# yang-z-03/scd-resnet

Hardware: AMD Instinct MI355X
Metric: 512x512 images/sec training, centerOffsetRes10, at 1/2/4/8 MI355X (higher is better)
Workload: dtype bf16; 1 GPU; centerOffsetRes10 train step (fwd+focal/L1 loss+bwd+Adam, DDP over RCCL), 512x512 synthetic SCD tiles; model=centerOffsetRes10, global_batch=32, step_issue=eager launches, per_gpu_batch=32, parallelism=dp1, image_size=512

## Files before the change

### include/scdhip.h

```cpp
#ifndef SCDHIP_H
#define SCDHIP_H
#include <stddef.h>
#include <stdint.h>

#ifdef __cplusplus
extern "C" {
#endif

#define SCD_DT_F32 0
#define SCD_DT_BF16 1
#define SCD_DT_F16 2

#define SCD_ERR_ARG 9001

#define SCD_MAX_TAPS 16
#define SCD_MAX_PHASES 4
#define SCD_STAT_REPLICAS 64

typedef struct scd_gemm_phase {
    int Qh, Qw, rho_h, rho_w, ntaps;
    int dh[SCD_MAX_TAPS], dw[SCD_MAX_TAPS], wt[SCD_MAX_TAPS];
} scd_gemm_phase;

int scd_conv_gemm(int dtype, const void* x, const void* w, void* y, const float* bias, double* stats,
                  int N, int Hi, int Wi, int Ci, int Ho, int Wo, int Co, int in_stride, int out_stride,
                  int wrow, int relu, int accumulate, int nphase, const scd_gemm_phase* phases,
                  void* stream);

int scd_conv_dgrad_s2(int dtype, const void* dy, const void* w3, void* dx, int N, int Hq, int Wq, int Cg, int Cin,
                      int accumulate, void* stream);
int scd_conv_gemm_bnbwd(int dtype, const void* x, const void* w, void* y, int N, int Hi, int Wi, int Ci, int Ho,
                        int Wo, int Co, int in_stride, int out_stride, int wrow, int nphase,
                        const scd_gemm_phase* phases, const void* bn_y, const float* mean, const float* invstd,
                        const float* relu_scale, const float* relu_shift, double* bn_stats, void* stream);
int scd_conv_gemm_heads(int dtype, const void* x, const void* w, void* hid, const float* bias, int N, int H,
                        int W, int Ci, int nh, const int* od, const float* const* w1, const float* const* b1,
                        float* const* outs, void* stream);
int scd_conv_gemm_heads_keep(int dtype, const void* x, const void* w, void* hid, const float* bias, int N, int H,
                             int W, int Ci, int nh, const int* od, const float* const* w1, const float* const* b1,
                             float* const* outs, const unsigned char* keep, int keep_cols, void* stream);

size_t scd_conv_wgrad_workspace(int Cg, int T, int Ci, int nsplit);
int scd_conv_wgrad_nsplit(int dtype, long M, int Cg, int T, int Ci);
int scd_conv_wgrad_nsplit2(int dtype, long M, int Ho, int Wo, int Cg, int T, int Ci);
int scd_conv_wgrad(int dtype, const void* g, const void* x, float* ws, int nsplit,
                   int N, int Ho, int Wo, int Cg, int Hi, int Wi, int Ci, int in_stride,
                   int T, const int* dh, const int* dw, void* stream);
int scd_wgrad_reduce(const float* ws, int nsplit, int Cg, int T, int Ci, int r0, int r1, int cvalid,
                     long ld_n, long ld_c, long ld_t, float* dst, int accumulate, float alpha, void* stream);
int scd_wgrad_reduce_rows(const float* ws, int nsplit, int Cg, int T, int Ci, int nslices, const int* r0,
                          const int* r1, const long* ld_n, const long* ld_c, const long* ld_t, float* const* dst,
                          int cvalid, int accumulate, float alpha, void* stream);

int scd_pack_weight(int dtype, const float* w, void* out, int A, int B, int T, int mode, int ldp,
                    int row_off, void* stream);

int scd_pad_channels(int dtype, const void* src, long rows, int C, int Cp, void* dst, void* stream);

typedef struct scd_pack_desc {
    const float* w;
    void* out;
    long start;
    int A, B, T, mode, ldp, row_off, a_off, a_tot;
} scd_pack_desc;
int scd_pack_weights_batched(int dtype, const scd_pack_desc* descs, int n, long total, void* stream);

int scd_im2col_stem(int dtype, const float* x, void* cols, int N, int H, int W, int Ho, int Wo, int kh,
                    int kw, int stride, int pad, int Kpad, void* stream);

int scd_stem_conv_fwd(int dtype, const float* x, const void* wpk, void* y, double* stats, int N, int H, int W,
                      int Ho, int Wo, void* stream);
int scd_stem_conv_wgrad_nsplit(long M);
int scd_stem_conv_wgrad(int dtype, const void* dy, const void* ybn, const float* coef, const float* x, float* ws,
                        int nsplit, int N, int H, int W, int Ho, int Wo, void* stream);
int scd_stem_bwd_nsplit(void);
int scd_stem_bwd_fused(int dtype, const void* dout, const uint8_t* argmax, const void* y, const float* scale,
                       const float* shift, const float* mean, const float* invstd, const float* x, double* stats,
                       float* ws, int nsplit, float* tg, int N, int H, int W, int Ho, int Wo, void* stream);
int scd_stem_bwd_combine(int dtype, const float* tg, const void* wpk, const float* coef, float* dst, int accumulate,
                         float alpha, void* stream);

int scd_stats_collapse(double* stats, int nrep, int C, void* stream);
int scd_stats_collapse_to(double* stats, int nrep, int C, double* out, void* stream);
int scd_bn_finalize(double* stats, int nrep, int C, double count, const float* gamma,
                    const float* beta, float* running_mean, float* running_var, int64_t* num_batches,
                    float momentum, float eps, float* mean, float* invstd, float* scale, float* shift,
                    void* stream);
#define SCD_BN_FIN_MAX 4
typedef struct scd_bn_fin_args {
    double* stats;
    int nrep, C;
    double count;
    const float* gamma;
    const float* beta;
    float* running_mean;
    float* running_var;
    int64_t* num_batches;
    float momentum, eps;
    float* mean;
    float* invstd;
    float* scale;
    float* shift;
} scd_bn_fin_args;
int scd_bn_finalize_n(const scd_bn_fin_args* layers, int n, void* stream);
int scd_bn_apply(int dtype, const void* y, void* out, int C, long total, const float* scale,
                 const float* shift, const void* res, const float* rscale, const float* rshift,
                 int relu, void* stream);
int scd_bn_bwd_reduce(int dtype, const void* dout, const void* mask, const void* y, const float* relu_scale,
                      const float* relu_shift, const float* mean, const float* invstd, int C, long total,
                      double* stats, void* stream);
int scd_bn_bwd_finalize(double* stats, int nrep, int C, double count, const float* gamma,
                        const float* mean, const float* invstd, float* dgamma, float* dbeta,
                        float gscale, float* coef, void* stream);
typedef struct scd_bn_bwd_fin_args {
    double* stats;
    int nrep, C;
    double count;
    const float* gamma;
    const float* mean;
    const float* invstd;
    float* dgamma;
    float* dbeta;
    float gscale;
    float* coef;
} scd_bn_bwd_fin_args;
int scd_bn_bwd_finalize_n(const scd_bn_bwd_fin_args* layers, int n, void* stream);
int scd_bn_bwd_apply(int dtype, const void* dout, const void* mask, const void* y, const float* relu_scale,
                     const float* relu_shift, const float* coef, int C, long total, void* dy, void* dz,
                     void* stream);

int scd_bn_bwd_reduce2(int dtype, const void* dout, const void* mask, const void* ya, const void* yb,
                       const float* mean_a, const float* invstd_a, const float* mean_b, const float* invstd_b, int C,
                       long total, double* stats_a, double* stats_b, void* stream);
int scd_bn_bwd_apply2(int dtype, const void* dout, const void* mask, const void* ya, const void* yb,
                      const float* coef_a, const float* coef_b, int C, long total, void* dya, void* dyb, void* stream);
// ... 122 lines not shown
```

### scd-resnet_amd/csrc/conv_gemm.hip

```cpp
#include <stdlib.h>

#include <algorithm>
#include <type_traits>

#include "scd_common.h"

#ifndef SCD_ABLATE
#define SCD_ABLATE 0
#endif
#ifndef L1P_SWAP
#define L1P_SWAP 1
#endif
#ifndef S1X1_FULLROW
#define S1X1_FULLROW 1
#endif
#ifndef S1X1_STG
#define S1X1_STG 1
#endif
#ifndef S1X1_UA2
#define S1X1_UA2 1
#endif
#ifndef WGRAD_OCC
#define WGRAD_OCC 2
#endif
// ... 3591 lines not shown
    fill_params(p, dy, w3, dx, nullptr, nullptr, N, Hq, Wq, Cg, Hq, Wq, Co, 1, 1, 4 * Cg, 0, accumulate);
    p.shuf = 1;
    scd_gemm_phase ph;
    ph.Qh = Hq; ph.Qw = Wq; ph.rho_h = 0; ph.rho_w = 0; ph.ntaps = 4;
    for (int t = 0; t < 4; ++t) { ph.dh[t] = t >> 1; ph.dw[t] = t & 1; ph.wt[t] = t; }
    return conv_gemm_launch(dtype, p, 1, &ph, stream);
}

extern "C" int scd_conv_gemm_heads(int dtype, const void* x, const void* w, void* hid, const float* bias, int N,
                                   int H, int W, int Ci, int nh, const int* od, const float* const* w1,
                                   const float* const* b1, float* const* outs, void* stream) {
    SCD_F16_FWD(scd_conv_gemm_heads, x, w, hid, bias, N, H, W, Ci, nh, od, w1, b1, outs, stream);
    return scd_conv_gemm_heads_keep(dtype, x, w, hid, bias, N, H, W, Ci, nh, od, w1, b1, outs, nullptr, 0, stream);
}

extern "C" int scd_conv_gemm_heads_keep(int dtype, const void* x, const void* w, void* hid, const float* bias, int N,
                                        int H, int W, int Ci, int nh, const int* od, const float* const* w1,
                                        const float* const* b1, float* const* outs, const unsigned char* keep,
                                        int keep_cols, void* stream) {
    SCD_F16_FWD(scd_conv_gemm_heads_keep, x, w, hid, bias, N, H, W, Ci, nh, od, w1, b1, outs, keep, keep_cols, stream);
    if (nh < 1 || nh > 4 || (keep && (keep_cols < 0 || keep_cols % 128))) return SCD_ERR_ARG;
    GemmParams p;
    fill_params(p, x, w, hid, bias, nullptr, N, H, W, Ci, H, W, nh * 128, 1, 1, 9 * Ci, 1, 0);
    if (keep) { p.hid_keep = keep; p.hid_cols = keep_cols; }
    p.head_on = 1;
    for (int h = 0; h < nh; ++h) {
        if (od[h] < 1 || od[h] > 4) return SCD_ERR_ARG;
        p.head_od[h] = od[h]; p.head_w[h] = w1[h]; p.head_b[h] = b1[h]; p.head_out[h] = outs[h];
    }
    scd_gemm_phase ph;
    ph.Qh = H; ph.Qw = W; ph.rho_h = 0; ph.rho_w = 0; ph.ntaps = 9;
    for (int t = 0; t < 9; ++t) { ph.dh[t] = t / 3 - 1; ph.dw[t] = t % 3 - 1; ph.wt[t] = t; }
    return conv_gemm_launch(dtype, p, 1, &ph, stream);
}

extern "C" size_t scd_conv_wgrad_workspace(int Cg, int T, int Ci, int nsplit) {
    return (size_t)nsplit * Cg * T * Ci * sizeof(float);
}

static bool wgrad_fastx() {
    static int mode = -2;
    if (mode == -2) { const char* e = getenv("SCD_WGRAD_FASTX"); mode = e ? atoi(e) : 1; }
    return mode != 0;
}

static void wgrad_tile(int dtype, long M, int Cg, int& tm, int& tn) {
    (void)dtype; (void)M;
    if (Cg <= 64) { tm = 64; tn = 256; }
    else { tm = 128; tn = 128; }
}

static bool wgrad_use_pp2(int dtype, long M, int Ho, int Wo, int Cg) {
    static int mode = -2;
    if (mode == -2) { const char* e = getenv("SCD_WGRAD_PP2"); mode = e ? atoi(e) : 1; }
    const bool stage_ok = Wo % 64 == 0 || (Wo >= 8 && 64 % Wo == 0);
    return mode && dtype == SCD_DT_BF16 && Cg >= 128 && stage_ok && ((long)Ho * Wo) % 64 == 0 && M >= 64 * 64;
}

static bool wgrad_use_l1(int dtype, long M, int Ho, int Wo, int Cg, int T, int Ci) {
    static int mode = -2;
    if (mode == -2) { const char* e = getenv("SCD_WGRAD_L1"); mode = e ? atoi(e) : 1; }
    return mode && dtype == SCD_DT_BF16 && Cg == 64 && Ci == 64 && T == 9 && Wo % 64 == 0 && M % 64 == 0 &&
           (long)Ho * Wo * 64 <= (1L << 30) && M >= 64;
}

static int wgrad_l1_nsplit(long M) {
    static long cap = -2;
    if (cap == -2) { const char* e = getenv("SCD_WGRAD_L1_NSPLIT"); cap = e ? atol(e) : 192; }
    return (int)std::max(1L, std::min(cap, M / 64 / 16));
}

static int wgrad_pp2_win(int Cg) {
    if (Cg % 256 == 0) return 256;
    if (Cg % 192 == 0) return 192;
    return Cg < 256 ? 128 : 256;
}

static bool wgrad_nsmodel() {
    static int mode = -2;
    if (mode == -2) { const char* e = getenv("SCD_WGRAD_NSMODEL"); mode = e ? atoi(e) : 1; }
    return mode != 0;
}

static long wgrad_ns_model(long M, long tiles, int slots, int kp, double stage_us, double epi_us, double slab_bytes,
                           long ns_max, bool any_ns = false) {
    static double slab_rate = -1.0;
    if (slab_rate < 0) { const char* e = getenv("SCD_WGRAD_SLAB_TBPS"); slab_rate = (e ? atof(e) : 0.8) * 1e6; }
    long best = 8;
    double bt = 1e30;
    const long step = any_ns ? 1 : 8;
    for (long ns = step; ns <= std::max(8L, ns_max); ns += step) {
        const long stages = cdiv(cdiv(M, ns), (long)kp);
        const long rounds = cdiv(tiles * ns, (long)slots);
        const double t = rounds * (stages * stage_us + epi_us) + ns * slab_bytes / slab_rate;
        if (t < bt * 0.995) { bt = t; best = ns; }
    }
    return best;
}

static int wgrad_pp2_nsplit(long M, int Cg, int KK) {
    const int win = wgrad_pp2_win(Cg);
    const long tiles = (long)(Cg / win) * cdiv(KK, 256);
    const long cap_px = std::max(8L, M / 512 / 8 * 8);
    const long cap_mem = std::max(8L, (256L << 20) / std::max(1L, 4L * Cg * KK) / 8 * 8);
    if (wgrad_nsmodel()) {
        const double stage_us = 2.0 * win * 256 * 64 / 4.3e6;
        const double epi_us = 4.0 * win * 256 / (5.0e6 / 256);
        static int slots = -1;
        if (slots < 0) { const char* e = getenv("SCD_WGRAD_SLOTS"); slots = e ? std::max(8, atoi(e)) : 256; }
        const long ns = wgrad_ns_model(M, tiles, slots, 64, stage_us, epi_us, 4.0 * Cg * KK, std::min(cap_px, cap_mem),
                                       tiles >= 24);
        return (int)ns;
    }
    long ns = std::max(8L, (512L / tiles + 4) / 8 * 8);
    ns = std::min(ns, cap_px);
    ns = std::min(ns, cap_mem);
    return (int)ns;
}

extern "C" int scd_conv_wgrad_nsplit2(int dtype, long M, int Ho, int Wo, int Cg, int T, int Ci) {
    SCD_F16_FWD(scd_conv_wgrad_nsplit2, M, Ho, Wo, Cg, T, Ci);
    if (wgrad_use_l1(dtype, M, Ho, Wo, Cg, T, Ci)) return wgrad_l1_nsplit(M);
    if (wgrad_use_pp2(dtype, M, Ho, Wo, Cg)) return wgrad_pp2_nsplit(M, Cg, T * Ci);
    return scd_conv_wgrad_nsplit(dtype, M, Cg, T, Ci);
}

extern "C" int scd_conv_wgrad_nsplit(int dtype, long M, int Cg, int T, int Ci) {
    SCD_F16_FWD(scd_conv_wgrad_nsplit, M, Cg, T, Ci);
    int tm, tn;
    wgrad_tile(dtype, M, Cg, tm, tn);
    const long tiles = (long)cdiv(Cg, tm) * cdiv((long)T * Ci, tn);
    if (wgrad_nsmodel() && M >= 8 * 1024) {
        const int KP = dtype == SCD_DT_BF16 ? 64 : 32;
        const int slots = tm == 64 ? 256 : 512;
        const double stage_us = 2.0 * tm * tn * KP / (2.4e6 * 256 / slots);
        const double epi_us = 4.0 * tm * tn / (5.0e6 / slots);
        const long cap_px = std::max(8L, M / 1024 / 8 * 8);
        const long cap_mem = std::max(8L, (256L << 20) / std::max(1L, 4L * Cg * T * Ci) / 8 * 8);
        const long ns = wgrad_ns_model(M, tiles, slots, KP, stage_us, epi_us, 4.0 * Cg * T * Ci,
                                       std::min(cap_px, cap_mem));
        return (int)ns;
    }
    long ns = std::max(1L, std::min(1024L / std::max(1L, tiles), M / 1024));
    ns = std::max(1L, std::min(ns, (256L << 20) / std::max(1L, 4L * Cg * T * Ci)));
    if (ns >= 8) ns = ns / 8 * 8;
    return (int)ns;
}

extern "C" int scd_conv_wgrad(int dtype, const void* g, const void* x, float* ws, int nsplit, int N, int Ho, int Wo,
                              int Cg, int Hi, int Wi, int Ci, int in_stride, int T, const int* dh, const int* dw,
                              void* stream) {
    SCD_F16_FWD(scd_conv_wgrad, g, x, ws, nsplit, N, Ho, Wo, Cg, Hi, Wi, Ci, in_stride, T, dh, dw, stream);
    const int EPC = dtype == SCD_DT_BF16 ? 8 : 4;
    if (T < 1 || T > SCD_MAX_TAPS || Ci % EPC != 0 || Cg % EPC != 0 || nsplit < 1) return SCD_ERR_ARG;
    WgradParams p;
    p.g = (const char*)g; p.x = (const char*)x; p.ws = ws;
    p.N = N; p.Ho = Ho; p.Wo = Wo; p.Cg = Cg; p.Hi = Hi; p.Wi = Wi; p.Ci = Ci; p.is = in_stride; p.T = T;
    p.cg0 = 0; p.cgn = Cg;
    p.KK = T * Ci;
    {
        const int esz = dtype == SCD_DT_BF16 ? 2 : 4;
        const long gb = (long)N * Ho * Wo * Cg * esz, xb = (long)N * Hi * Wi * Ci * esz;
        if (gb >= (1L << 31) - 64 || xb >= (1L << 31) - 64) return SCD_ERR_ARG;
        p.gbytes = (int)gb;
        p.xbytes = (int)xb;
    }
    for (int t = 0; t < SCD_MAX_TAPS; ++t) { p.dh[t] = t < T ? dh[t] : 0; p.dw[t] = t < T ? dw[t] : 0; }
    const long M = (long)N * Ho * Wo;
    int chunk = cdiv(M, nsplit);
    chunk = (chunk + 63) / 64 * 64;
    p.chunk = chunk;
    if (wgrad_use_l1(dtype, M, Ho, Wo, Cg, T, Ci) && in_stride == 1 && Hi == Ho && Wi == Wo) {
        bool std_taps = true;
        for (int t = 0; t < 9; ++t) std_taps &= dh[t] == t / 3 - 1 && dw[t] == t % 3 - 1;
        if (std_taps) {
            p.nsplit = nsplit;
            hipLaunchKernelGGL(conv_wgrad_l1_kernel, dim3(nsplit), dim3(512), 0, (hipStream_t)stream, p);
            SCD_RETURN_LAUNCH();
        }
    }
    if (wgrad_use_pp2(dtype, M, Ho, Wo, Cg) && chunk % 64 == 0) {
        hipStream_t st = (hipStream_t)stream;
        p.ntn = cdiv(p.KK, 256);
        p.nsplit = nsplit;
        const int n8 = nsplit;
        const int win = wgrad_pp2_win(Cg);
        p.cg0 = 0;
        p.cgn = Cg / win * win;
        p.ntm = Cg / win;
        if (win == 256) hipLaunchKernelGGL((conv_wgrad_pp2_kernel<4>), dim3(p.ntm * p.ntn * n8), dim3(512), 0, st, p);
        else if (win == 192) hipLaunchKernelGGL((conv_wgrad_pp2_kernel<3>), dim3(p.ntm * p.ntn * n8), dim3(512), 0, st, p);
        else hipLaunchKernelGGL((conv_wgrad_pp2_kernel<2>), dim3(p.ntm * p.ntn * n8), dim3(512), 0, st, p);
        hipError_t e = hipGetLastError();
        if (e != hipSuccess || Cg % win == 0) return (int)e;
// ... 4 lines not shown
        p.ntm = cdiv(p.cgn, BM);
        p.ntn = cdiv(p.KK, BN);
        const int fx = !(wgrad_fastx() && ((long)Ho * Wo) % 64 == 0) ? 0 : (Wo % 64 == 0 ? 1 : 2);
        dim3 grid(p.ntm * p.ntn * n8);
        if (BM == 64) {
            if (fx == 1) hipLaunchKernelGGL((conv_wgrad_kernel<h16, 64, 256, 1>), grid, dim3(256), 0, st, p);
            else if (fx == 2) hipLaunchKernelGGL((conv_wgrad_kernel<h16, 64, 256, 2>), grid, dim3(256), 0, st, p);
            else hipLaunchKernelGGL((conv_wgrad_kernel<h16, 64, 256, 0>), grid, dim3(256), 0, st, p);
        } else {
            if (fx == 1) hipLaunchKernelGGL((conv_wgrad_kernel<h16, 128, 128, 1>), grid, dim3(256), 0, st, p);
            else hipLaunchKernelGGL((conv_wgrad_kernel<h16, 128, 128, 0>), grid, dim3(256), 0, st, p);
        }
        SCD_RETURN_LAUNCH();
    }
    int BM, BN;
    wgrad_tile(dtype, M, Cg, BM, BN);
    p.ntm = cdiv(Cg, BM);
    p.ntn = cdiv(p.KK, BN);
    p.nsplit = nsplit;
    dim3 grid(p.ntm * p.ntn * nsplit);
    hipStream_t st = (hipStream_t)stream;
    if (dtype == SCD_DT_BF16 || dtype == SCD_DT_F32) {
        const int KP = dtype == SCD_DT_BF16 ? 64 : 32;
        const bool fastok = wgrad_fastx() && ((long)Ho * Wo) % KP == 0 && chunk % KP == 0;
        const int fx = !fastok ? 0 : (Wo % KP == 0 ? 1 : (KP % Wo == 0 ? 2 : 0));
        if (dtype == SCD_DT_BF16) {
            if (Cg <= 64) {
                if (fx == 1) hipLaunchKernelGGL((conv_wgrad_kernel<h16, 64, 256, 1>), grid, dim3(256), 0, st, p);
                else if (fx == 2) hipLaunchKernelGGL((conv_wgrad_kernel<h16, 64, 256, 2>), grid, dim3(256), 0, st, p);
                else hipLaunchKernelGGL((conv_wgrad_kernel<h16, 64, 256, 0>), grid, dim3(256), 0, st, p);
            } else {
                if (fx == 1) hipLaunchKernelGGL((conv_wgrad_kernel<h16, 128, 128, 1>), grid, dim3(256), 0, st, p);
                else hipLaunchKernelGGL((conv_wgrad_kernel<h16, 128, 128, 0>), grid, dim3(256), 0, st, p);
            }
        } else {
            if (Cg <= 64) {
                if (fx == 1) hipLaunchKernelGGL((conv_wgrad_kernel<float, 64, 256, 1>), grid, dim3(256), 0, st, p);
                else if (fx == 2) hipLaunchKernelGGL((conv_wgrad_kernel<float, 64, 256, 2>), grid, dim3(256), 0, st, p);
                else hipLaunchKernelGGL((conv_wgrad_kernel<float, 64, 256, 0>), grid, dim3(256), 0, st, p);
            } else {
                if (fx == 1) hipLaunchKernelGGL((conv_wgrad_kernel<float, 128, 128, 1>), grid, dim3(256), 0, st, p);
                else hipLaunchKernelGGL((conv_wgrad_kernel<float, 128, 128, 0>), grid, dim3(256), 0, st, p);
            }
        }
    } else {
        return SCD_ERR_ARG;
    }
    SCD_RETURN_LAUNCH();
}

extern "C" int scd_wgrad_reduce_rows(const float* ws, int nsplit, int Cg, int T, int Ci, int nslices, const int* r0,
                                     const int* r1, const long* ld_n, const long* ld_c, const long* ld_t,
                                     float* const* dst, int cvalid, int accumulate, float alpha, void* stream) {
    if (nslices < 1 || nslices > 4 || nsplit < 1 || Ci % 4 != 0 || T < 1 || T > 64) return SCD_ERR_ARG;
    WredSlices sl;
    sl.n = nslices;
    long rows = 0;
    for (int s = 0; s < nslices; ++s) {
        if (r0[s] < 0 || r1[s] > Cg || r0[s] >= r1[s] || dst[s] == nullptr) return SCD_ERR_ARG;
        sl.r0[s] = r0[s]; sl.r1[s] = r1[s];
        sl.ldn[s] = ld_n[s]; sl.ldc[s] = ld_c[s]; sl.ldt[s] = ld_t[s];
        sl.dst[s] = dst[s];
        rows += r1[s] - r0[s];
    }
    const long zs = (long)Cg * T * Ci;
    int cb = WRED_CB;
    while (cb > 16 && rows * cdiv(Ci, cb) < 512) cb >>= 1;
    const int ncb = cdiv(Ci, cb);
    const int units = T * (std::min(cb, Ci) / 4);
    const int S = std::max(1, std::min(256 / std::max(1, units), nsplit / 8));
    const int threads = (int)std::min(256L, ((long)units * S + 63) / 64 * 64);
    const size_t lds = (size_t)((T * (cb + 1) + 3) & ~3) * sizeof(float) + (S > 1 ? (size_t)S * units * 16 : 0);
    hipLaunchKernelGGL(wgrad_reduce_kernel, dim3((unsigned)(rows * ncb)), dim3(threads), lds, (hipStream_t)stream, ws,
                       nsplit, zs, T, Ci, cvalid, sl, ncb, cb, S, accumulate, alpha);
    SCD_RETURN_LAUNCH();
}

extern "C" int scd_wgrad_reduce(const float* ws, int nsplit, int Cg, int T, int Ci, int r0, int r1, int cvalid,
                                long ld_n, long ld_c, long ld_t, float* dst, int accumulate, float alpha,
                                void* stream) {
    return scd_wgrad_reduce_rows(ws, nsplit, Cg, T, Ci, 1, &r0, &r1, &ld_n, &ld_c, &ld_t, &dst, cvalid, accumulate,
                                 alpha, stream);
}
```

### scd-resnet_amd/scdhip/lib.py

```python
import ctypes
import os

import torch

HERE = os.path.dirname(os.path.abspath(__file__))
LIB_PATH = os.environ.get("SCDHIP_LIB", os.path.join(HERE, "libscdhip.so"))

DT_F32 = 0
DT_BF16 = 1
DT_F16 = 2
MAX_TAPS = 16
MAX_PHASES = 4
STAT_REPLICAS = 64

c_int, c_long, c_float, c_double, c_size_t, c_void_p = (ctypes.c_int, ctypes.c_long, ctypes.c_float,
                                                        ctypes.c_double, ctypes.c_size_t, ctypes.c_void_p)


class GemmPhase(ctypes.Structure):
    _fields_ = [("Qh", c_int), ("Qw", c_int), ("rho_h", c_int), ("rho_w", c_int), ("ntaps", c_int),
                ("dh", c_int * MAX_TAPS), ("dw", c_int * MAX_TAPS), ("wt", c_int * MAX_TAPS)]


class BnFinArgs(ctypes.Structure):
    _fields_ = [("stats", c_void_p), ("nrep", c_int), ("C", c_int), ("count", c_double), ("gamma", c_void_p),
                ("beta", c_void_p), ("running_mean", c_void_p), ("running_var", c_void_p), ("num_batches", c_void_p),
                ("momentum", c_float), ("eps", c_float), ("mean", c_void_p), ("invstd", c_void_p), ("scale", c_void_p),
                ("shift", c_void_p)]


class BnBwdFinArgs(ctypes.Structure):
    _fields_ = [("stats", c_void_p), ("nrep", c_int), ("C", c_int), ("count", c_double), ("gamma", c_void_p),
                ("mean", c_void_p), ("invstd", c_void_p), ("dgamma", c_void_p), ("dbeta", c_void_p),
                ("gscale", c_float), ("coef", c_void_p)]


class PackDesc(ctypes.Structure):
    _fields_ = [("w", c_void_p), ("out", c_void_p), ("start", c_long), ("A", c_int), ("B", c_int), ("T", c_int),
                ("mode", c_int), ("ldp", c_int), ("row_off", c_int), ("a_off", c_int), ("a_tot", c_int)]


P = c_void_p
I = c_int
L = c_long
F = c_float
D = c_double
PP = ctypes.POINTER(c_void_p)
IP = ctypes.POINTER(c_int)
LP = ctypes.POINTER(c_long)

SIGNATURES = {
    "scd_conv_gemm": (I, [I, P, P, P, P, P, I, I, I, I, I, I, I, I, I, I, I, I, I, ctypes.POINTER(GemmPhase), P]),
    "scd_conv_gemm_heads": (I, [I, P, P, P, P, I, I, I, I, I, IP, PP, PP, PP, P]),
    "scd_conv_gemm_heads_keep": (I, [I, P, P, P, P, I, I, I, I, I, IP, PP, PP, PP, P, I, P]),
    "scd_conv_gemm_bnbwd": (I, [I, P, P, P, I, I, I, I, I, I, I, I, I, I, I, ctypes.POINTER(GemmPhase), P, P, P, P,
                                P, P, P]),
    "scd_conv_wgrad_workspace": (c_size_t, [I, I, I, I]),
    "scd_conv_wgrad_nsplit": (I, [I, L, I, I, I]),
    "scd_conv_wgrad_nsplit2": (I, [I, L, I, I, I, I, I]),
    "scd_conv_wgrad": (I, [I, P, P, P, I, I, I, I, I, I, I, I, I, I, IP, IP, P]),
    "scd_wgrad_reduce": (I, [P, I, I, I, I, I, I, I, L, L, L, P, I, F, P]),
    "scd_wgrad_reduce_rows": (I, [P, I, I, I, I, I, IP, IP, LP, LP, LP, PP, I, I, F, P]),
    "scd_pack_weight": (I, [I, P, P, I, I, I, I, I, I, P]),
    "scd_pack_weights_batched": (I, [I, P, I, L, P]),
    "scd_pad_channels": (I, [I, P, L, I, I, P, P]),
    "scd_im2col_stem": (I, [I, P, P, I, I, I, I, I, I, I, I, I, I, P]),
    "scd_stem_conv_fwd": (I, [I, P, P, P, P, I, I, I, I, I, P]),
    "scd_stem_conv_wgrad_nsplit": (I, [L]),
    "scd_stem_conv_wgrad": (I, [I, P, P, P, P, P, I, I, I, I, I, I, P]),
    "scd_stem_bwd_nsplit": (I, []),
    "scd_conv_dgrad_s2": (I, [I, P, P, P, I, I, I, I, I, I, P]),
    "scd_stem_bwd_fused": (I, [I, P, P, P, P, P, P, P, P, P, P, I, P, I, I, I, I, I, P]),
    "scd_stem_bwd_combine": (I, [I, P, P, P, P, I, F, P]),
    "scd_stem_pool_bwd_bn": (I, [I, P, P, P, P, P, P, P, P, P, I, I, I, I, I, I, P]),
    "scd_stats_collapse": (I, [P, I, I, P]),
    "scd_stats_collapse_to": (I, [P, I, I, P, P]),
    "scd_bn_finalize": (I, [P, I, I, D, P, P, P, P, P, F, F, P, P, P, P, P]),
    "scd_bn_apply": (I, [I, P, P, I, L, P, P, P, P, P, I, P]),
    "scd_bn_bwd_reduce": (I, [I, P, P, P, P, P, P, P, I, L, P, P]),
    "scd_bn_bwd_finalize": (I, [P, I, I, D, P, P, P, P, P, F, P, P]),
    "scd_bn_finalize_n": (I, [ctypes.POINTER(BnFinArgs), I, P]),
    "scd_bn_bwd_finalize_n": (I, [ctypes.POINTER(BnBwdFinArgs), I, P]),
    "scd_bn_bwd_apply": (I, [I, P, P, P, P, P, P, I, L, P, P, P]),
    "scd_bn_bwd_reduce2": (I, [I, P, P, P, P, P, P, P, P, I, L, P, P, P]),
    "scd_bn_bwd_apply2": (I, [I, P, P, P, P, P, P, I, L, P, P, P]),
    "scd_stem_pool_fwd": (I, [I, P, P, P, P, P, I, I, I, I, I, I, P]),
    "scd_stem_pool_bwd": (I, [I, P, P, P, P, P, P, I, I, I, I, I, I, P]),
    "scd_heads_fwd": (I, [I, P, I, I, I, I, IP, PP, PP, PP, P]),
    "scd_heads_bwd_accsize": (c_size_t, [I, I, IP]),
    "scd_heads_bwd": (I, [I, P, I, I, I, I, IP, PP, PP, P, P, P]),
    "scd_heads_bwd_packed": (I, [I, P, I, I, I, I, IP, PP, PP, F, P, P, P, P]),
    "scd_heads_bwd_weight_finalize": (I, [P, I, I, IP, PP, PP, PP, I, F, P]),
    "scd_heads_bwd_packed_split": (I, [I, P, I, I, I, I, IP, I, PP, PP, F, P, P, P, P]),
    "scd_heads_sparse_bwd": (I, [I, P, P, I, I, I, I, I, I, IP, I, PP, PP, F, P, I, P, P, P, P, P, P]),
    "scd_heads_sparse_fixup": (I, [I, P, P, I, I, I, I, P, I, P, P, P, P, P, P, P, P, P]),
    "scd_focal_fwd": (I, [P, P, L, P, P, P]),
    "scd_l1_gather_fwd": (I, [P, I, I, I, P, P, P, I, I, I, P, P, P]),
    "scd_centernet_loss_finalize": (I, [P, I, P, I, P, P, P, P]),
    "scd_scale_by_device": (I, [P, L, P, I, P, P]),
    "scd_heads_keep_map": (I, [P, I, I, I, P, I, P, P]),
    "scd_centernet_loss_fwd": (I, [P, P, L, P, I, P, I, I, I, P, P, P, I, I, I, I, P, P, P, P, P, P, P, P]),
    "scd_centernet_loss_bwd_scale": (I, [P, L, I, I, P, I, P, I, P, I, P, P, P]),
    "scd_decode_workspace": (c_size_t, [I, I]),
    "scd_decode_topk": (I, [P, I, I, I, I, P, I, P, I, P, P, P, P, P, P, P, P]),
    "scd_augment_workspace": (c_size_t, [I]),
    "scd_augment_tiles": (I, [P, P, I, I, I, P, P, P, F, ctypes.c_ulonglong, P, P]),
    "scd_slide_workspace": (c_size_t, [I]),
    "scd_slide_tiles": (I, [P, I, I, I, I, I, I, I, I, I, I, P, P, P]),
    "scd_slide_detections": (I, [P, I, I, I, I, I, I, F, P, P, P, P]),
    "scd_slide_rotate_workspace": (c_size_t, [I, I]),
    "scd_slide_rotate_clips": (I, [P, I, I, I, I, I, I, I, I, ctypes.POINTER(c_double), I, P, P, P]),
    "scd_ceval_count": (I, [P, P, P, P, P, P, P, I, I, I, I, I, I, F, P, P]),
    "scd_ceval_emit": (I, [P, P, P, P, P, P, P, I, I, I, I, I, I, F, P, PP, P]),
    "scd_ceval_summary_workspace": (c_size_t, [L]),
    "scd_ceval_summary": (I, [PP, ctypes.POINTER(c_long), L, P, I, P, P, P]),
    "scd_adam_step": (I, [P, P, P, P, L, F, F, F, F, F, F, F, P]),
    "scd_adam_step_dev": (I, [P, P, P, P, L, P, F, F, F, F, P, P]),
    "scd_sgd_step_dev": (I, [P, P, P, L, P, F, F, F, I, F, P, P]),
    "scd_render_center_targets": (I, [P, P, I, I, I, F, P, P, P, P, P]),
    "scd_cpool_fwd": (I, [I, I, P, P, P, I, I, I, I, P]),
    "scd_cpool_bwd": (I, [I, I, P, P, P, I, I, I, I, P]),
    "scd_nms": (I, [P, L, I, I, I, P, P]),
    "scd_topk": (I, [P, I, L, I, I, I, P, P, P, P, P, P]),
    "scd_focal_prob_fwd": (I, [P, P, L, P, P, P]),
    "scd_masked_l1_fwd": (I, [P, P, P, L, I, I, P, P, P]),
    "scd_peer_mailbox_bytes": (c_size_t, [I, I]),
    "scd_peer_alloc": (I, [c_size_t, PP]),
    "scd_peer_free": (I, [P]),
    "scd_peer_ipc_handle": (I, [P, P]),
    "scd_peer_ipc_open": (I, [P, PP]),
    "scd_peer_ipc_close": (I, [P]),
    "scd_peer_allreduce_f64": (I, [P, I, I, I, PP, I, ctypes.c_ulonglong, P, ctypes.c_uint, P]),
    "scd_event_create": (I, [PP]),
    "scd_event_destroy": (I, [P]),
    "scd_event_record": (I, [P, P]),
    "scd_event_elapsed_ms": (I, [P, P, ctypes.POINTER(c_float)]),
    "scd_calib_mfma_peak": (I, [P, I, I, P, P, P]),
    "scd_calib_set_stamps": (I, [P]),
    "scd_calib_stamped_build": (I, []),
    "scd_version": (ctypes.c_char_p, []),
}


class _Lib:
    def __init__(self, path):
# ... 58 lines not shown
```

### scd-resnet_amd/scdhip/ops.py

```python
import contextlib
import ctypes
import math
import os

import torch
import torch.distributed as dist

from . import lib as L

_DT = {torch.float32: L.DT_F32, torch.bfloat16: L.DT_BF16, torch.float16: L.DT_F16}
HALF = (torch.bfloat16, torch.float16)


class LossScale:
    f16 = float(os.environ.get("SCD_F16_LOSS_SCALE", "1024"))
    scaled_task = None


def loss_scale(dtype):
    return LossScale.f16 if dtype == torch.float16 else 1.0


def begin_loss_scale(dtype):
    S = loss_scale(dtype)
# ... 778 lines not shown

class _Side:
    enabled = os.environ.get("SCD_WGRAD_STREAM", "1") != "0"
    batch = None
    priority = 10
    streams = {}
    joined_task = {}


def _graph_task():
    try:
        return torch._C._current_graph_task_id()
    except Exception:
        return -1


def side_stream(dev):
    task = _graph_task()
    if not _Side.enabled or task == -1:
        return None
    idx = dev.index if dev.index is not None else torch.cuda.current_device()
    s = _Side.streams.get(idx)
    if s is None:
        s = _new_side_stream(idx)
        _Side.streams[idx] = s
    if _Side.batch is None or idx not in _Side.batch:
        s.wait_stream(torch.cuda.current_stream(idx))
        if _Side.batch is not None:
            _Side.batch.add(idx)
    if _Side.joined_task.get(idx) != task:
        _Side.joined_task[idx] = task
        torch.autograd.Variable._execution_engine.queue_callback(join_side_streams)
    return s


def _new_side_stream(idx):
    return torch.cuda.Stream(device=idx, priority=_Side.priority)


@contextlib.contextmanager
def side_batch():
    outer = _Side.batch
    _Side.batch = set() if outer is None else outer
    try:
        yield
    finally:
        _Side.batch = outer


def join_side_streams():
    for idx, s in _Side.streams.items():
        torch.cuda.current_stream(idx).wait_stream(s)
    _Side.joined_task.clear()


def side_stream_for_comm(dev):
    idx = dev.index if dev.index is not None else torch.cuda.current_device()
    s = _Side.streams.get(idx)
    if s is None or _graph_task() == -1:
        return None
    s.wait_stream(torch.cuda.current_stream(idx))
    return s


def conv_wgrad(g, x, kh, kw, stride, pad, dst, ld, cvalid=None, accumulate=True, rows=None, red_taps=1):
    _conv_wgrad_side(g, x, kh, kw, stride, pad, dst, ld, cvalid, accumulate, rows, red_taps)


def _conv_wgrad_side(g, x, kh, kw, stride, pad, dst, ld, cvalid=None, accumulate=True, rows=None, red_taps=1):
    side = side_stream(g.device) if g.is_cuda else None
    if side is None:
        return _conv_wgrad(g, x, kh, kw, stride, pad, dst, ld, cvalid, accumulate, rows, red_taps)
    with torch.cuda.stream(side):
        _conv_wgrad(g, x, kh, kw, stride, pad, dst, ld, cvalid, accumulate, rows, red_taps)
    g.record_stream(side)
    x.record_stream(side)


def _conv_wgrad(g, x, kh, kw, stride, pad, dst, ld, cvalid=None, accumulate=True, rows=None, red_taps=1):
    N, Ho, Wo, Cg = g.shape
    _, Hi, Wi, Ci = x.shape
    T = kh * kw
    d = dt(g)
    key = (d, N, Ho, Wo, Cg, Ci, kh, kw, pad)
    plan = _WGRAD_PLANS.get(key)
    if plan is None:
        dh = L.int_array([r - pad for r in range(kh) for s in range(kw)])
        dw = L.int_array([s - pad for r in range(kh) for s in range(kw)])
        ns = L.lib().scd_conv_wgrad_nsplit2(d, N * Ho * Wo, Ho, Wo, Cg, T, Ci)
        plan = _WGRAD_PLANS[key] = (dh, dw, ns, L.lib().scd_conv_wgrad_workspace(Cg, T, Ci, ns) // 4)
    dh, dw, ns, wsn = plan
    ws = torch.empty(wsn, dtype=torch.float32, device=g.device)
    t0 = ClassTimer.begin()
    L.call("scd_conv_wgrad", d, ptr(g), ptr(x), ptr(ws), ns, N, Ho, Wo, Cg, Hi, Wi, Ci, stride, T, dh, dw, stream())
    if rows is None:
        rows = [(0, Cg, dst, ld)]
    Tr, Cr = T * red_taps, Ci // red_taps
    cv = Cr if cvalid is None else cvalid
    for i in range(0, len(rows), 4):
        part = rows[i:i + 4]
        rkey = tuple((r[0], r[1], ptr(r[2]), tuple(r[3])) for r in part)
        arrs = _WGRAD_ROWS.get(rkey)
        if arrs is None:
            if len(_WGRAD_ROWS) > 4096:
                _WGRAD_ROWS.clear()
            arrs = _WGRAD_ROWS[rkey] = (
                L.int_array([r[0] for r in part]), L.int_array([r[1] for r in part]),
                L.long_array([r[3][0] for r in part]), L.long_array([r[3][1] for r in part]),
                L.long_array([r[3][2] for r in part]), L.ptr_array([ptr(r[2]) for r in part]))
        L.call("scd_wgrad_reduce_rows", ptr(ws), ns, Cg, Tr, Cr, len(part), *arrs, cv, int(accumulate), grad_alpha(g),
               stream())
    if t0 is not None:
        ClassTimer.end("wgrad", t0, 2.0 * N * Ho * Wo * Cg * T * Ci)


_WGRAD_PLANS = {}
_WGRAD_ROWS = {}



class BNState:
    __slots__ = ("mean", "invstd", "scale", "shift", "count")


def bn_finalize(bn, stats, C, count, training=True):
    st = _bn_state(C, bn.weight.device)
    if training:
        return _bn_finalize_launch(bn, st, stats, _allreduce_stats(stats, C), C, count)
    else:
        L.call("scd_bn_finalize", 0, 0, C, 1.0, ptr(bn.weight), ptr(bn.bias), ptr(bn.running_mean),
               ptr(bn.running_var), 0, 0.0, float(bn.eps), ptr(st.mean), ptr(st.invstd), ptr(st.scale),
               ptr(st.shift), stream())
    st.count = count
    return st


def _bn_finalize_launch(bn, st, stats, nrep, C, count):
    count = count * bn_sync_world()
    L.call("scd_bn_finalize", ptr(stats), nrep, C, float(count), ptr(bn.weight), ptr(bn.bias),
           ptr(bn.running_mean), ptr(bn.running_var), ptr(bn.num_batches_tracked), float(bn.momentum),
           float(bn.eps), ptr(st.mean), ptr(st.invstd), ptr(st.scale), ptr(st.shift), stream())
    st.count = count
    return st


def _bn_state(C, dev):
    st = BNState()
    st.mean, st.invstd, st.scale, st.shift = torch.empty(4, C, device=dev).unbind(0)
    return st


def bn_finalize_pair(bn_a, stats_a, Ca, count_a, bn_b, stats_b, Cb, count_b):
    sa, sb, nrep = _allreduce_stats_pair(stats_a, Ca, stats_b, Cb)
    sts, args = [], (L.BnFinArgs * 2)()
    for i, (bn, stats, C, count) in enumerate(((bn_a, sa, Ca, count_a), (bn_b, sb, Cb, count_b))):
        st = _bn_state(C, bn.weight.device)
        st.count = count * bn_sync_world()
        args[i] = L.BnFinArgs(ptr(stats), nrep, C, float(st.count), ptr(bn.weight), ptr(bn.bias), ptr(bn.running_mean),
                              ptr(bn.running_var), ptr(bn.num_batches_tracked), float(bn.momentum), float(bn.eps),
                              ptr(st.mean), ptr(st.invstd), ptr(st.scale), ptr(st.shift))
        sts.append(st)
    L.call("scd_bn_finalize_n", args, 2, stream())
    return sts[0], sts[1]


def bn_apply(y, st, relu, res=None, rst=None, out=None):
    C = y.shape[-1]
    if out is None:
        out = torch.empty_like(y)
    t0 = ClassTimer.begin()
    L.call("scd_bn_apply", dt(y), ptr(y), ptr(out), C, y.numel(), ptr(st.scale), ptr(st.shift), ptr(res),
           ptr(rst.scale) if rst is not None else 0, ptr(rst.shift) if rst is not None else 0, int(relu), stream())
    if t0 is not None:
        ClassTimer.end("bn", t0, y.numel() * y.element_size() * (3 if res is not None else 2))
    return out


def bn_backward(bn, st, dout, y, mask=None, dz_out=None, relu=False, stats=None):
    C = y.shape[-1]
    rsc, rsh = (ptr(st.scale), ptr(st.shift)) if (relu and mask is None) else (0, 0)
    E = y.numel() * y.element_size()
    if stats is None:
        stats = bn_stats(bn, "bwd")
        t0 = ClassTimer.begin()
        L.call("scd_bn_bwd_reduce", dt(y), ptr(dout), ptr(mask), ptr(y), rsc, rsh, ptr(st.mean), ptr(st.invstd),
               C, y.numel(), ptr(stats), stream())
        if t0 is not None:
            ClassTimer.end("bn", t0, E * (3 if mask is not None else 2))
    coef = bn_backward_coef(bn, st, stats, C, grad_alpha(y))
    dy = torch.empty_like(y)
    t0 = ClassTimer.begin()
    L.call("scd_bn_bwd_apply", dt(y), ptr(dout), ptr(mask), ptr(y), rsc, rsh, ptr(coef), C, y.numel(), ptr(dy),
           ptr(dz_out), stream())
    if t0 is not None:
        ClassTimer.end("bn", t0, E * (3 + (mask is not None) + (dz_out is not None)))
    return dy
# ... 337 lines not shown
```

Measured before the change: 6120 images/s.

## Add transposed-orientation wgrad path chosen by cost model for stride-1 convs

Adds a planning entry point that can compute the weight gradient in transposed orientation, swapping the roles of input activations and output gradient and negating tap offsets, when the convolution is stride-1, same-size, bf16 and writes the whole weight. A cost model compares both orientations for Cg==128 with Ci>Cg and picks the transposed one only when it is predicted to be clearly cheaper. The reduce step then writes through swapped leading dimensions, so no extra transpose kernel is needed. Risks are wrong gradients if the swapped strides or negated offsets are off, and a mispredicting model.

```diff
diff --git a/include/scdhip.h b/include/scdhip.h
--- a/include/scdhip.h
+++ b/include/scdhip.h
@@ -51,6 +51,14 @@
 int scd_wgrad_reduce_rows(const float* ws, int nsplit, int Cg, int T, int Ci, int nslices, const int* r0,
                           const int* r1, const long* ld_n, const long* ld_c, const long* ld_t, float* const* dst,
                           int cvalid, int accumulate, float alpha, void* stream);
+int scd_conv_wgrad_plan(int dtype, int N, int Ho, int Wo, int Cg, int Hi, int Wi, int Ci, int in_stride, int T,
+                        const int* dh, const int* dw, int whole, int orient_in, int* orient, int* nsplit,
+                        size_t* ws_bytes);
+int scd_conv_wgrad_to(int dtype, const void* g, const void* x, float* ws, size_t ws_bytes, int N, int Ho, int Wo,
+                      int Cg, int Hi, int Wi, int Ci, int in_stride, int T, const int* dh, const int* dw,
+                      int orient_in, int nslices, const int* r0, const int* r1, const long* ld_n, const long* ld_c,
+                      const long* ld_t, float* const* dst, int cvalid, int red_taps, int accumulate, float alpha,
+                      void* stream);
 
 int scd_pack_weight(int dtype, const float* w, void* out, int A, int B, int T, int mode, int ldp,
                     int row_off, void* stream);
diff --git a/scd-resnet_amd/csrc/conv_gemm.hip b/scd-resnet_amd/csrc/conv_gemm.hip
--- a/scd-resnet_amd/csrc/conv_gemm.hip
+++ b/scd-resnet_amd/csrc/conv_gemm.hip
@@ -3697,23 +3697,32 @@
     return mode != 0;
 }
 
+static double wgrad_slab_rate() {
+    static double slab_rate = -1.0;
+    if (slab_rate < 0) { const char* e = getenv("SCD_WGRAD_SLAB_TBPS"); slab_rate = (e ? atof(e) : 0.8) * 1e6; }
+    return slab_rate;
+}
+
+static double wgrad_ns_cost(long M, long tiles, int slots, int kp, double stage_us, double epi_us, double slab_bytes,
+                            long ns) {
+    const long stages = cdiv(cdiv(M, ns), (long)kp);
+    const long rounds = cdiv(tiles * ns, (long)slots);
+    return rounds * (stages * stage_us + epi_us) + ns * slab_bytes / wgrad_slab_rate();
+}
+
 static long wgrad_ns_model(long M, long tiles, int slots, int kp, double stage_us, double epi_us, double slab_bytes,
                            long ns_max, bool any_ns = false) {
-    static double slab_rate = -1.0;
-    if (slab_rate < 0) { const char* e = getenv("SCD_WGRAD_SLAB_TBPS"); slab_rate = (e ? atof(e) : 0.8) * 1e6; }
     long best = 8;
     double bt = 1e30;
     const long step = any_ns ? 1 : 8;
     for (long ns = step; ns <= std::max(8L, ns_max); ns += step) {
-        const long stages = cdiv(cdiv(M, ns), (long)kp);
-        const long rounds = cdiv(tiles * ns, (long)slots);
-        const double t = rounds * (stages * stage_us + epi_us) + ns * slab_bytes / slab_rate;
+        const double t = wgrad_ns_cost(M, tiles, slots, kp, stage_us, epi_us, slab_bytes, ns);
         if (t < bt * 0.995) { bt = t; best = ns; }
     }
     return best;
 }
 
-static int wgrad_pp2_nsplit(long M, int Cg, int KK) {
+static int wgrad_pp2_nsplit(long M, int Cg, int KK, bool any_ns = false, int tr_slots = 0) {
     const int win = wgrad_pp2_win(Cg);
     const long tiles = (long)(Cg / win) * cdiv(KK, 256);
     const long cap_px = std::max(8L, M / 512 / 8 * 8);
@@ -3723,8 +3732,9 @@
         const double epi_us = 4.0 * win * 256 / (5.0e6 / 256);
         static int slots = -1;
         if (slots < 0) { const char* e = getenv("SCD_WGRAD_SLOTS"); slots = e ? std::max(8, atoi(e)) : 256; }
-        const long ns = wgrad_ns_model(M, tiles, slots, 64, stage_us, epi_us, 4.0 * Cg * KK, std::min(cap_px, cap_mem),
-                                       tiles >= 24);
+        const long ns = wgrad_ns_model(M, tiles, tr_slots > 0 ? tr_slots : slots, 64, stage_us, epi_us, 4.0 * Cg * KK,
+                                       std::min(cap_px, cap_mem),
+                                       tiles >= 24 || any_ns);
         return (int)ns;
     }
     long ns = std::max(8L, (512L / tiles + 4) / 8 * 8);
@@ -3895,3 +3905,94 @@
     return scd_wgrad_reduce_rows(ws, nsplit, Cg, T, Ci, 1, &r0, &r1, &ld_n, &ld_c, &ld_t, &dst, cvalid, accumulate,
                                  alpha, stream);
 }
+
+#ifndef SCD_F16_BUILD
+static bool wgrad_tr_eligible(int d16, long M, int Ho, int Wo, int Cg, int Hi, int Wi, int Ci, int in_stride, int T,
+                              int whole) {
+    if (d16 != SCD_DT_BF16 || in_stride != 1 || Hi != Ho || Wi != Wo || !whole) return false;
+    if (wgrad_use_l1(d16, M, Ho, Wo, Cg, T, Ci)) return false;
+    if (!wgrad_use_pp2(d16, M, Ho, Wo, Ci) || Ci % wgrad_pp2_win(Ci) != 0) return false;
+    return (long)M * Ci * 2 < (1L << 31) - 64 && (long)M * Cg * 2 < (1L << 31) - 64;
+}
+
+#ifndef SCD_WGRAD_TR_ANYNS
+#define SCD_WGRAD_TR_ANYNS 0
+#endif
+#ifndef SCD_WGRAD_TR_SLOTS
+#define SCD_WGRAD_TR_SLOTS 160
+#endif
+#ifndef SCD_WGRAD_TR_MARGIN
+#define SCD_WGRAD_TR_MARGIN 0.9
+#endif
+static double wgrad_pp2_model_cu_us(long M, int Cw, int KK, int ns) {
+    const int win = wgrad_pp2_win(Cw);
+    const long tiles = (long)(Cw / win) * cdiv(KK, 256);
+    const double rate = win == 256 ? 4.3e6 : win == 192 ? 3.5e6 : 2.8e6;
+    const double stage_us = 2.0 * win * 256 * 64 / rate, epi_us = 4.0 * win * 256 / (5.0e6 / 256);
+    const long stages = cdiv(cdiv(M, (long)ns), 64L);
+    return (double)tiles * ns * (stages * stage_us + epi_us) + 256.0 * ns * (4.0 * Cw * KK) / wgrad_slab_rate();
+}
+
+extern "C" int scd_conv_wgrad_plan(int dtype, int N, int Ho, int Wo, int Cg, int Hi, int Wi, int Ci, int in_stride,
+                                   int T, const int* dh, const int* dw, int whole, int orient_in, int* orient,
+                                   int* nsplit, size_t* ws_bytes) {
+    const int EPC = dtype == SCD_DT_F32 ? 4 : 8;
+    if ((dtype != SCD_DT_F32 && dtype != SCD_DT_BF16 && dtype != SCD_DT_F16) || N < 1 || Ho < 1 || Wo < 1 || Hi < 1 ||
+        Wi < 1 || Cg < 1 || Ci < 1 || in_stride < 1 || T < 1 || T > SCD_MAX_TAPS || Ci % EPC != 0 || Cg % EPC != 0 ||
+        !dh || !dw || orient_in < -1 || orient_in > 1 || !orient || !nsplit || !ws_bytes)
+        return SCD_ERR_ARG;
+    const long M = (long)N * Ho * Wo;
+    const int d16 = dtype == SCD_DT_F16 ? SCD_DT_BF16 : dtype;
+    const int ns0 = scd_conv_wgrad_nsplit2(dtype, M, Ho, Wo, Cg, T, Ci);
+    int o = 0, ns = ns0;
+    if (orient_in != 0 && wgrad_tr_eligible(d16, M, Ho, Wo, Cg, Hi, Wi, Ci, in_stride, T, whole)) {
+        const int ns1 = wgrad_pp2_nsplit(M, Ci, T * Cg, SCD_WGRAD_TR_ANYNS != 0, SCD_WGRAD_TR_SLOTS);
+        if (orient_in == 1) {
+            o = 1;
+        } else if (Cg == 128 && Ci > Cg && wgrad_use_pp2(d16, M, Ho, Wo, Cg)) {
+            o = wgrad_pp2_model_cu_us(M, Ci, T * Cg, ns1) <
+                SCD_WGRAD_TR_MARGIN * wgrad_pp2_model_cu_us(M, Cg, T * Ci, ns0);
+        }
+        if (o) ns = ns1;
+    }
+    *orient = o;
+    *nsplit = ns;
+    *ws_bytes = scd_conv_wgrad_workspace(Cg, T, Ci, ns);
+    return 0;
+}
+
+extern "C" int scd_conv_wgrad_to(int dtype, const void* g, const void* x, float* ws, size_t ws_bytes, int N, int Ho,
+                                 int Wo, int Cg, int Hi, int Wi, int Ci, int in_stride, int T, const int* dh,
+                                 const int* dw, int orient_in, int nslices, const int* r0, const int* r1,
+                                 const long* ld_n, const long* ld_c, const long* ld_t, float* const* dst, int cvalid,
+                                 int red_taps, int accumulate, float alpha, void* stream) {
+    if (!g || !x || !ws || nslices < 1 || !r0 || !r1 || !ld_n || !ld_c || !ld_t || !dst || red_taps < 1 ||
+        Ci % std::max(1, red_taps) != 0 || (long)T * red_taps > 64)
+        return SCD_ERR_ARG;
+    const int Tr = T * red_taps, Cr = Ci / red_taps;
+    if (cvalid < 1 || cvalid > Cr) return SCD_ERR_ARG;
+    for (int s = 0; s < nslices; ++s)
+        if (r0[s] < 0 || r1[s] > Cg || r0[s] >= r1[s] || !dst[s]) return SCD_ERR_ARG;
+    const int whole = nslices == 1 && r0[0] == 0 && r1[0] == Cg && red_taps == 1 && cvalid == Ci;
+    int orient, ns;
+    size_t need;
+    int rc = scd_conv_wgrad_plan(dtype, N, Ho, Wo, Cg, Hi, Wi, Ci, in_stride, T, dh, dw, whole, orient_in, &orient, &ns,
+                                 &need);
+    if (rc) return rc;
+    if (ws_bytes < need) return SCD_ERR_ARG;
+    if (orient) {
+        int ndh[SCD_MAX_TAPS], ndw[SCD_MAX_TAPS];
+        for (int t = 0; t < T; ++t) { ndh[t] = -dh[t]; ndw[t] = -dw[t]; }
+        rc = scd_conv_wgrad(dtype, x, g, ws, ns, N, Hi, Wi, Ci, Ho, Wo, Cg, 1, T, ndh, ndw, stream);
+        if (rc) return rc;
+        const int z0 = 0;
+        return scd_wgrad_reduce_rows(ws, ns, Ci, T, Cg, 1, &z0, &Ci, ld_c, ld_n, ld_t, dst, Cg, accumulate, alpha,
+                                     stream);
+    }
+    rc = scd_conv_wgrad(dtype, g, x, ws, ns, N, Ho, Wo, Cg, Hi, Wi, Ci, in_stride, T, dh, dw, stream);
+    for (int s = 0; s < nslices && !rc; s += 4)
+        rc = scd_wgrad_reduce_rows(ws, ns, Cg, Tr, Cr, std::min(4, nslices - s), r0 + s, r1 + s, ld_n + s, ld_c + s,
+                                   ld_t + s, dst + s, cvalid, accumulate, alpha, stream);
+    return rc;
+}
+#endif
diff --git a/scd-resnet_amd/scdhip/lib.py b/scd-resnet_amd/scdhip/lib.py
--- a/scd-resnet_amd/scdhip/lib.py
+++ b/scd-resnet_amd/scdhip/lib.py
@@ -61,6 +61,9 @@
     "scd_conv_wgrad": (I, [I, P, P, P, I, I, I, I, I, I, I, I, I, I, IP, IP, P]),
     "scd_wgrad_reduce": (I, [P, I, I, I, I, I, I, I, L, L, L, P, I, F, P]),
     "scd_wgrad_reduce_rows": (I, [P, I, I, I, I, I, IP, IP, LP, LP, LP, PP, I, I, F, P]),
+    "scd_conv_wgrad_plan": (I, [I, I, I, I, I, I, I, I, I, I, IP, IP, I, I, IP, IP, ctypes.POINTER(c_size_t)]),
+    "scd_conv_wgrad_to": (I, [I, P, P, P, c_size_t, I, I, I, I, I, I, I, I, I, IP, IP, I, I, IP, IP, LP, LP, LP, PP, I,
+                              I, I, F, P]),
     "scd_pack_weight": (I, [I, P, P, I, I, I, I, I, I, P]),
     "scd_pack_weights_batched": (I, [I, P, I, L, P]),
     "scd_pad_channels": (I, [I, P, L, I, I, P, P]),
diff --git a/scd-resnet_amd/scdhip/ops.py b/scd-resnet_amd/scdhip/ops.py
--- a/scd-resnet_amd/scdhip/ops.py
+++ b/scd-resnet_amd/scdhip/ops.py
@@ -884,36 +884,43 @@
     _, Hi, Wi, Ci = x.shape
     T = kh * kw
     d = dt(g)
-    key = (d, N, Ho, Wo, Cg, Ci, kh, kw, pad)
+    if rows is None:
+        rows = [(0, Cg, dst, ld)]
+    cv = Ci // red_taps if cvalid is None else cvalid
+    whole = int(len(rows) == 1 and rows[0][0] == 0 and rows[0][1] == Cg and red_taps == 1 and cv == Ci)
+    key = (d, N, Ho, Wo, Cg, Hi, Wi, Ci, kh, kw, stride, pad, whole)
     plan = _WGRAD_PLANS.get(key)
     if plan is None:
         dh = L.int_array([r - pad for r in range(kh) for s in range(kw)])
         dw = L.int_array([s - pad for r in range(kh) for s in range(kw)])
-        ns = L.lib().scd_conv_wgrad_nsplit2(d, N * Ho * Wo, Ho, Wo, Cg, T, Ci)
-        plan = _WGRAD_PLANS[key] = (dh, dw, ns, L.lib().scd_conv_wgrad_workspace(Cg, T, Ci, ns) // 4)
-    dh, dw, ns, wsn = plan
-    ws = torch.empty(wsn, dtype=torch.float32, device=g.device)
+        orient_in = _wgrad_orient()
+        o, ns, wsb = L.c_int(), L.c_int(), L.c_size_t()
+        L.call("scd_conv_wgrad_plan", d, N, Ho, Wo, Cg, Hi, Wi, Ci, stride, T, dh, dw, whole, orient_in,
+               ctypes.byref(o), ctypes.byref(ns), ctypes.byref(wsb))
+        plan = _WGRAD_PLANS[key] = (dh, dw, orient_in, wsb.value)
+    dh, dw, orient_in, wsb = plan
+    ws = torch.empty(wsb // 4, dtype=torch.float32, device=g.device)
     t0 = ClassTimer.begin()
-    L.call("scd_conv_wgrad", d, ptr(g), ptr(x), ptr(ws), ns, N, Ho, Wo, Cg, Hi, Wi, Ci, stride, T, dh, dw, stream())
-    if rows is None:
-        rows = [(0, Cg, dst, ld)]
-    Tr, Cr = T * red_taps, Ci // red_taps
-    cv = Cr if cvalid is None else cvalid
-    for i in range(0, len(rows), 4):
-        part = rows[i:i + 4]
-        rkey = tuple((r[0], r[1], ptr(r[2]), tuple(r[3])) for r in part)
-        arrs = _WGRAD_ROWS.get(rkey)
-        if arrs is None:
-            if len(_WGRAD_ROWS) > 4096:
-                _WGRAD_ROWS.clear()
-            arrs = _WGRAD_ROWS[rkey] = (
-                L.int_array([r[0] for r in part]), L.int_array([r[1] for r in part]),
-                L.long_array([r[3][0] for r in part]), L.long_array([r[3][1] for r in part]),
-                L.long_array([r[3][2] for r in part]), L.ptr_array([ptr(r[2]) for r in part]))
-        L.call("scd_wgrad_reduce_rows", ptr(ws), ns, Cg, Tr, Cr, len(part), *arrs, cv, int(accumulate), grad_alpha(g),
-               stream())
+    rkey = tuple((r[0], r[1], ptr(r[2]), tuple(r[3])) for r in rows)
+    arrs = _WGRAD_ROWS.get(rkey)
+    if arrs is None:
+        if len(_WGRAD_ROWS) > 4096:
+            _WGRAD_ROWS.clear()
+        arrs = _WGRAD_ROWS[rkey] = (
+            L.int_array([r[0] for r in rows]), L.int_array([r[1] for r in rows]),
+            L.long_array([r[3][0] for r in rows]), L.long_array([r[3][1] for r in rows]),
+            L.long_array([r[3][2] for r in rows]), L.ptr_array([ptr(r[2]) for r in rows]))
+    L.call("scd_conv_wgrad_to", d, ptr(g), ptr(x), ptr(ws), wsb, N, Ho, Wo, Cg, Hi, Wi, Ci, stride, T, dh, dw,
+           orient_in, len(rows), *arrs, cv, red_taps, int(accumulate), grad_alpha(g), stream())
     if t0 is not None:
         ClassTimer.end("wgrad", t0, 2.0 * N * Ho * Wo * Cg * T * Ci)
+
+
+def _wgrad_orient():
+    v = os.environ.get("SCD_WGRAD_ORIENT", "auto")
+    if v not in ("auto", "0", "1"):
+        raise ValueError("SCD_WGRAD_ORIENT must be auto, 0 or 1, not %r" % v)
+    return -1 if v == "auto" else int(v)
 
 
 _WGRAD_PLANS = {}
```

New measurement: 6174 images/s, median of 6. Within noise of the previous version (+0.9%).
